# michaelosthege/pytensor-federated

Measured on NVIDIA H100. Metric: logp+grad evals/sec for 8-shard federated GLM, higher is better.
Workload: dtype bf16; 1 GPU; model=federated logistic GLM (logp + gradient), chains_per_eval=1, features=256, global_batch=80000000, seq_len=256, l2_policy=inputs (>= 2.5 GB per GPU) are larger than the 50 MB L2; no flush needed, parallelism=shard-parallel x1 (8 shards/GPU), kernel=auto, backend=fused, comm=local, hbm_bytes_per_eval_per_gpu=31200395264

## Files before the change

### pytensor_federated_b200/csrc/fed_comm.cuh

```cuda
#pragma once
#include <cstdint>
#include <cuda_runtime.h>

#define B200FED_MAX_WORLD 8

#define B200FED_STATUS_SHIFT 56
#define B200FED_EPOCH_MASK 0x00FFFFFFFFFFFFFFull
#define B200FED_ERR_THETA_TIMEOUT 1ull
#define B200FED_ERR_PEER_TIMEOUT 2ull
#define B200FED_ERR_PIPELINE 4ull
#define B200FED_STOP_EPOCH 0x00FFFFFFFFFFFFFFull

struct FedComm {
    int rank;
    int world;
    int n_theta;
    int n_vals;
    unsigned long long epoch;
    unsigned long long timeout_ns;

    const float* theta_src;
    float* peer_theta[B200FED_MAX_WORLD];
    unsigned long long* peer_flag[B200FED_MAX_WORLD];
    float* mc_theta;
// ... 215 lines not shown
        return rl;
    }
    if (c.rank == 0 && blockIdx.x == 0) {
        for (int i = threadIdx.x; i < c.n_theta; i += blockDim.x) {
            float v = c.theta_src[i];
            if (c.mc_theta) {
                multimem_st_f32(c.mc_theta + i, v);
            } else {
                for (int p = 0; p < c.world; ++p) c.peer_theta[p][i] = v;
            }
        }
        __threadfence_system();
        __syncthreads();
        if (threadIdx.x == 0 && c.trace) c.trace[(epoch & 255) * 4 + 0] = globaltimer();
        if (c.mc_flag) {
            if (threadIdx.x == 0) multimem_st_release_u64(c.mc_flag, epoch);
        } else if (threadIdx.x < c.world) {
            st_release_sys(c.peer_flag[threadIdx.x], epoch);
        }
    }
    if (threadIdx.x == 0) {
        unsigned long long seen = 0;
        s_ok = wait_epoch(c.flag_local, epoch, c.timeout_ns, &seen) ? 1 : 0;
        s_seen = seen;
    }
    __syncthreads();
    Prologue r;
    r.epoch = epoch;
    r.timed_out = (s_ok == 0);
    r.stop = ((s_seen & B200FED_EPOCH_MASK) == B200FED_STOP_EPOCH);
    if (!r.timed_out && !r.stop) {
        for (int i = threadIdx.x; i < c.n_theta; i += blockDim.x) theta_smem[i] = ld_cg_f32(c.theta_local + i);
    }
    __syncthreads();
    if (threadIdx.x == 0) stamp(c, 1);
    return r;
}

__device__ __forceinline__ void dd_add(double& hi, double& lo, double xh, double xl) {
    const double s = hi + xh;
    const double bb = s - hi;
    const double err = (hi - (s - bb)) + (xh - bb);
    hi = s;
    lo += err + xl;
}
__device__ __forceinline__ double2 ld_cg_f64x2(const double* p) {
    double2 v;
    asm volatile("ld.global.cg.v2.f64 {%0, %1}, [%2];" : "=d"(v.x), "=d"(v.y) : "l"(p) : "memory");
    return v;
}

constexpr unsigned int kReduceGroup = 16;

template <bool DD>
__device__ __forceinline__ void sum_rows(const double* rows, size_t stride, int v, unsigned int first, unsigned int count,
                                         double& hi, double& lo) {
    constexpr unsigned int kWide = DD ? 16 : 37;
    hi = 0.0;
    lo = 0.0;
    for (unsigned int b = 0; b < count; b += kWide) {
        if constexpr (DD) {
            double2 t[kWide];
#pragma unroll
            for (unsigned int j = 0; j < kWide; ++j)
                t[j] = (b + j < count) ? ld_cg_f64x2(rows + (size_t)(first + b + j) * stride + 2 * (size_t)v) : make_double2(0.0, 0.0);
#pragma unroll
            for (unsigned int j = 0; j < kWide; ++j) dd_add(hi, lo, t[j].x, t[j].y);
        } else {
            double t[kWide];
#pragma unroll
            for (unsigned int j = 0; j < kWide; ++j)
                t[j] = (b + j < count) ? ld_cg_f64(rows + (size_t)(first + b + j) * stride + v) : 0.0;
#pragma unroll
            for (unsigned int j = 0; j < kWide; ++j) hi += t[j];
        }
    }
}

template <bool DD>
__device__ __forceinline__ bool epilogue_t(const FedComm& c, const Prologue& pro, unsigned long long status_in,
                                           size_t row_stride, double* group_buf) {
    __shared__ int s_last;
    __shared__ unsigned long long s_status;
    const int nv = c.n_vals;
    if (c.world == 1 && gridDim.x == 1) {
        __syncthreads();
        if (pro.timed_out || pro.stop) {
            if (threadIdx.x == 0) {
                if (pro.timed_out && !pro.stop && c.spec_theta && c.idle_ticks) {
                    volatile unsigned long long* ticks = c.idle_ticks;
                    *ticks = *ticks + 1ull;
                } else if (c.host_flag) {
                    __threadfence_system();
                    st_release_sys(c.host_flag, (pro.stop ? B200FED_STOP_EPOCH : pro.epoch) |
                                                    ((pro.stop ? 0ull : B200FED_ERR_THETA_TIMEOUT) << B200FED_STATUS_SHIFT));
                }
            }
            return true;
        }
        auto value = [&](int v) { return DD ? c.cta_partials[2 * v] + c.cta_partials[2 * v + 1] : c.cta_partials[v]; };
        if (c.ll_mode) {
            for (int v = threadIdx.x; v < nv; v += blockDim.x) ll_store_f64(c.ll_host_result + 2 * v, value(v), pro.epoch);
            if (threadIdx.x == 0) {
                if (c.trace) {
                    c.trace[(pro.epoch & 255) * 4 + 1] = globaltimer();
                    c.trace[(pro.epoch & 255) * 4 + 2] = globaltimer();
                }
                if (c.epoch_counter) *c.epoch_counter = pro.epoch;
                if (c.done_flag) *reinterpret_cast<volatile unsigned long long*>(c.done_flag) = pro.epoch;
                stamp(c, 7);
            }
            return true;
        }
        for (int v = threadIdx.x; v < nv; v += blockDim.x) c.host_result[v] = value(v);
        __threadfence_system();
        __syncthreads();
        if (threadIdx.x == 0) {
            if (c.trace) {
                c.trace[(pro.epoch & 255) * 4 + 1] = globaltimer();
                c.trace[(pro.epoch & 255) * 4 + 2] = globaltimer();
            }
            st_release_sys(c.host_flag, pro.epoch | (status_in << B200FED_STATUS_SHIFT));
            if (c.epoch_counter) *c.epoch_counter = pro.epoch;
            if (c.done_flag) *reinterpret_cast<volatile unsigned long long*>(c.done_flag) = pro.epoch;
            stamp(c, 7);
        }
        return true;
    }
    const bool computed = !(pro.stop || pro.timed_out);
    const unsigned int n_groups = (gridDim.x + kReduceGroup - 1) / kReduceGroup;
    const unsigned int grp = blockIdx.x / kReduceGroup;
    const unsigned int grp_first = grp * kReduceGroup;
    const unsigned int grp_size = min(kReduceGroup, gridDim.x - grp_first);
    constexpr int kW = DD ? 2 : 1;

    const unsigned long long status_cta = status_in | ((pro.timed_out && !pro.stop) ? B200FED_ERR_THETA_TIMEOUT : 0ull);
    if (threadIdx.x == 0 && status_cta) atomicOr(c.ticket + 255, (unsigned int)status_cta);
    __threadfence();
    __syncthreads();
    if (threadIdx.x == 0) {
        const unsigned int t = atomicAdd(c.ticket + 1 + grp, 1u);
        s_last = (t == grp_size - 1) ? 1 : 0;
        if (s_last) c.ticket[1 + grp] = 0;
        s_status = status_in;
    }
    __syncthreads();
    if (!s_last) {
        if (threadIdx.x == 0) stamp(c, 7);
        return false;
    }
    __threadfence();
    if (computed) {
        for (int v = threadIdx.x; v < nv; v += blockDim.x) {
            double hi, lo;
            sum_rows<DD>(c.cta_partials, row_stride, v, grp_first, grp_size, hi, lo);
            group_buf[((size_t)grp * nv + v) * kW] = hi;
            if constexpr (DD) group_buf[((size_t)grp * nv + v) * kW + 1] = lo;
        }
    }
    __threadfence();
    __syncthreads();
    if (threadIdx.x == 0) {
        const unsigned int t = atomicAdd(c.ticket, 1u);
        s_last = (t == n_groups - 1) ? 1 : 0;
    }
    __syncthreads();
    if (!s_last) {
        if (threadIdx.x == 0) stamp(c, 7);
        return false;
    }
    __threadfence();
    const unsigned long long epoch = pro.epoch;
    if (threadIdx.x == 0) {
        s_status |= (unsigned long long)atomicExch(c.ticket + 255, 0u);
    }
    __syncthreads();
    const bool any_timed_out = (s_status & B200FED_ERR_THETA_TIMEOUT) != 0ull;

    if (!computed || any_timed_out) {
        if (threadIdx.x == 0) {
            const bool timed_out = pro.timed_out || any_timed_out;
            const bool idle = timed_out && !pro.stop && (c.rank != 0 || c.spec_theta != nullptr);
            if (idle && c.rank == 0) *c.spec_abort = 0ull;
            const unsigned long long done_epoch = idle ? epoch - 1ull : epoch;
            *c.ticket = 0;
            if (c.epoch_counter) *c.epoch_counter = done_epoch;
            unsigned long long st = (timed_out && !idle) ? B200FED_ERR_THETA_TIMEOUT : 0ull;
            unsigned long long word = (pro.stop ? B200FED_STOP_EPOCH : done_epoch) | (st << B200FED_STATUS_SHIFT);
            if (idle && c.idle_ticks) {
                volatile unsigned long long* ticks = c.idle_ticks;
                *ticks = *ticks + 1ull;
            }
            if (c.done_flag) { *reinterpret_cast<volatile unsigned long long*>(c.done_flag) = word; }
            if (c.rank == 0 && c.host_flag) {
                __threadfence_system();
                st_release_sys(c.host_flag, word);
            }
        }
        return true;
    }
    auto node_value = [&](int v) {
        double hi, lo;
        sum_rows<DD>(group_buf, (size_t)nv * kW, v, 0u, n_groups, hi, lo);
        return hi + lo;
    };

    if (c.ll_mode) {
        unsigned long long* my_slot_ll = c.ll_root_slots + (size_t)c.rank * nv * 2;
        for (int v = threadIdx.x; v < nv; v += blockDim.x) {
            const double s = node_value(v);
            if (c.rank != 0) {
                ll_store_f64(my_slot_ll + 2 * v, s, epoch);
            } else {
                double total = s;
                bool ok = true;
                for (int p = 1; p < c.world && ok; ++p) {
                    unsigned int lo = 0, hi = 0;
                    const unsigned long long* src = c.ll_root_slots + ((size_t)p * nv + v) * 2;
                    ok = ll_wait_word(src, epoch, c.timeout_ns, nullptr, &lo) == 0 &&
                         ll_wait_word(src + 1, epoch, c.timeout_ns, nullptr, &hi) == 0;
                    total += __longlong_as_double((long long)(((unsigned long long)hi << 32) | lo));
                }
                if (ok) ll_store_f64(c.ll_host_result + 2 * v, total, epoch);
                else atomicOr(&s_status, B200FED_ERR_PEER_TIMEOUT);
            }
        }
        __syncthreads();
        if (threadIdx.x == 0) {
            if (c.trace) {
                c.trace[(epoch & 255) * 4 + 1] = globaltimer();
                if (c.rank == 0) c.trace[(epoch & 255) * 4 + 2] = globaltimer();
            }
            if (c.rank == 0 && s_status) {
                __threadfence_system();
                st_release_sys(c.host_flag, epoch | (s_status << B200FED_STATUS_SHIFT));
            }
            *c.ticket = 0;
            if (c.epoch_counter) *c.epoch_counter = epoch;
            if (c.done_flag) *reinterpret_cast<volatile unsigned long long*>(c.done_flag) = epoch | (s_status << B200FED_STATUS_SHIFT);
            stamp(c, 7);
        }
        return true;
    }

    if (c.rank != 0) {
        double* my_slot = c.root_slots + (size_t)c.rank * nv;
        for (int v = threadIdx.x; v < nv; v += blockDim.x) my_slot[v] = node_value(v);
        __threadfence_system();
        __syncthreads();
        if (threadIdx.x == 0) {
            if (c.trace) c.trace[(epoch & 255) * 4 + 1] = globaltimer();
            st_release_sys(c.root_slot_flags + c.rank, epoch);
        }
    } else {
        if (threadIdx.x == 0 && c.trace) c.trace[(epoch & 255) * 4 + 1] = globaltimer();
        constexpr int kOwn = 4;
// ... 72 lines not shown
```

### pytensor_federated_b200/csrc/glm_tc.cu

```cuda
#include <cstring>
#include <vector>

#include <cuda.h>
#include <cuda_bf16.h>
#include <cuda_runtime.h>

#include "fed_comm.cuh"
#include "models.h"
#include "tc_common.cuh"
#include "chunks.h"

namespace tc {

constexpr int kTileM = 128;
constexpr int kPanel = 64;
constexpr int kPanelBytes = kTileM * 128;
constexpr int kThreads = 384;
constexpr int kConsumerWarps = 8;
constexpr int kMaxChunk = 32;
constexpr int kMinChunk = 4;
constexpr int kRing = 16;
constexpr int kLLRows = 16;

constexpr int kXBlock = kTileM * kPanel * 3 / 2;
constexpr int kXFoot = 256;
constexpr int kXMaxExceptions = kXFoot / 4 - 1;
constexpr int kXSlots = 6;
constexpr int kDecThreads = 96;

__host__ __device__ __forceinline__ uint32_t x12_prmt(uint32_t a, uint32_t b, uint32_t s) {
#ifdef __CUDA_ARCH__
    uint32_t r;
    asm("prmt.b32 %0, %1, %2, %3;" : "=r"(r) : "r"(a), "r"(b), "r"(s));
    return r;
#else
    const uint64_t v = (uint64_t)b << 32 | a;
    uint32_t r = 0;
    for (int k = 0; k < 4; ++k) {
        const uint32_t sel = (s >> (4 * k)) & 0xFu;
        uint32_t byte = (uint32_t)(v >> (8 * (sel & 7u))) & 0xFFu;
        if (sel & 8u) byte = (byte & 0x80u) ? 0xFFu : 0u;
        r |= byte << (8 * k);
    }
    return r;
#endif
}
__host__ __device__ __forceinline__ uint4 x12_decode8(uint2 lo, uint32_t c, const uint32_t (&t)[4]) {
    const uint32_t w = c << 4;
    const uint32_t s0 = c & 0x7777u, s1 = (c >> 16) & 0x7777u;
    const uint32_t m0 = x12_prmt(w, c, 0xD9C8u), m1 = x12_prmt(w, c, 0xFBEAu);
    const uint32_t h0 = (x12_prmt(t[0], t[1], s0) & ~m0) | (x12_prmt(t[2], t[3], s0) & m0);
    const uint32_t h1 = (x12_prmt(t[0], t[1], s1) & ~m1) | (x12_prmt(t[2], t[3], s1) & m1);
    uint4 r;
    r.x = x12_prmt(lo.x, h0, 0x5140u);
    r.y = x12_prmt(lo.x, h0, 0x7362u);
    r.z = x12_prmt(lo.y, h1, 0x5140u);
    r.w = x12_prmt(lo.y, h1, 0x7362u);
    return r;
}
__host__ __device__ __forceinline__ uint32_t x12_chunk_offset(int i) { return (i >> 3) * 128 + (((i & 7) ^ ((i >> 3) & 7)) << 4); }
__host__ __device__ __forceinline__ uint32_t x12_high_byte_offset(uint32_t pos) {
    const uint32_t pnl = pos >> 13, row = (pos >> 6) & 127, f = pos & 63;
    return pnl * kPanelBytes + row * 128 + ((((f >> 3) ^ (row & 7)) << 4) | ((f & 7) << 1)) + 1;
}

struct SmemLayout {
    uint32_t stages, stage_bytes, off_theta_b, theta_b_bytes, off_r, r_bytes, off_rows, row_bytes, off_theta_f,
        off_disp, off_ring, off_bars, total, preload, xslots, xslot_bytes, off_x, off_xfoot;
};
__host__ __device__ inline SmemLayout smem_layout(int P, int n1, int n2, int n_theta, int chain_words, int chains,
                                                  int row_arrays, bool packed = false) {
    SmemLayout L;
    const uint32_t panels = P / kPanel;
    L.stage_bytes = panels * kPanelBytes;
    L.theta_b_bytes = panels * n1 * 128;
    L.r_bytes = kTileM * n2 * 2;
    L.row_bytes = (uint32_t)row_arrays * kTileM * 4;
    const uint32_t bars_bytes = packed ? 256 : 192;
    const uint32_t fixed = L.theta_b_bytes + 2 * L.r_bytes + ((chains * (1 + chain_words) * 4 + 15) & ~15) + kRing * 24 +
                           bars_bytes + (packed ? 2 * kXFoot : 0) + 1024 ;
    uint32_t stages = (227u * 1024u - fixed) / (L.stage_bytes + L.row_bytes);
// ... 156 lines not shown
            if (ROWS && segs_g[i].weight) tma_prefetch_desc(&tmaps[4 * i + 3]);
        }
    auto load_tile = [&](int st, int seg, int row0, int rows) {
        const CUtensorMap* m = tmaps + 4 * seg;
        float* slot = reinterpret_cast<float*>(smem + L.off_rows + (size_t)st * L.row_bytes);
        mbar_expect_tx(&bar_full[st], L.stage_bytes + kTileM * 4 * (1 + (rows & 1) + (rows >> 1)));
        for (int pnl = 0; pnl < panels; ++pnl)
            tma_load_2d(smem + (size_t)st * L.stage_bytes + pnl * kPanelBytes, m, pnl * kPanel, row0, &bar_full[st]);
        tma_load_1d(slot, m + 1, row0, &bar_full[st]);
        if (rows & 1) tma_load_1d(slot + o_slot * kTileM, m + 2, row0, &bar_full[st]);
        if (rows & 2) tma_load_1d(slot + w_slot * kTileM, m + 3, row0, &bar_full[st]);
    };
    auto load_xpanel = [&](int xs, int seg, int tile, int pnl, int rows) {
        unsigned char* dst = smem + L.off_x + (size_t)xs * L.xslot_bytes;
        const GlmSegment& g = segs_g[seg];
        const uint32_t extra = pnl == 0 ? kXFoot + kTileM * 4 * (1 + (rows & 1) + (rows >> 1)) : 0;
        mbar_expect_tx(&bar_xfull[xs], kXBlock + extra);
        bulk_load(dst, static_cast<const unsigned char*>(g.xpack) + ((size_t)tile * panels + pnl) * kXBlock, kXBlock, &bar_xfull[xs]);
        if (pnl == 0) {
            const CUtensorMap* m = tmaps + 4 * seg;
            float* slot = reinterpret_cast<float*>(dst + kXBlock + kXFoot);
            bulk_load(dst + kXBlock, static_cast<const unsigned char*>(g.xfoot) + (size_t)tile * kXFoot, kXFoot, &bar_xfull[xs]);
            tma_load_1d(slot, m + 1, tile * kTileM, &bar_xfull[xs]);
            if (rows & 1) tma_load_1d(slot + o_slot * kTileM, m + 2, tile * kTileM, &bar_xfull[xs]);
            if (rows & 2) tma_load_1d(slot + w_slot * kTileM, m + 3, tile * kTileM, &bar_xfull[xs]);
        }
    };
    auto seg_row_mask = [&](int seg) -> int {
        if constexpr (!ROWS) return 0;
        return (segs_g[seg].offset ? 1 : 0) | (segs_g[seg].weight ? 2 : 0);
    };
    unsigned int claim0 = 0;
    int preloaded = 0;
    if (warp == 0) {
        __syncwarp();
        fed::pdl_wait();
        if (lane == 0) claim0 = atomicAdd(work_counter, 1u);
        claim0 = __shfl_sync(0xffffffffu, claim0, 0);
        if (claim0 < (unsigned int)n_chunks) {
            const GlmChunk ch = chunks[claim0];
            const int units = PK ? ch.n_tiles * panels : ch.n_tiles;
            preloaded = units < (int)L.preload ? units : (int)L.preload;
            if (!prm.early_loads) preloaded = 0;
            const int rows = seg_row_mask(ch.seg);
            if (elect_one())
                for (int t = 0; t < preloaded; ++t) {
                    if (PK) load_xpanel(t, ch.seg, ch.first_tile + t / panels, t % panels, rows);
                    else load_tile(t, ch.seg, (ch.first_tile + t) * kTileM, rows);
                }
            __syncwarp();
        }
    }

    fed::Prologue pro = fed::prologue(comm, theta_f);
    const bool active = !pro.stop && !pro.timed_out;
    const int NOUT = prm.n_out;
    const int NS1 = 1 + G + DISP;
    const size_t row_doubles = partial_row_doubles(comm.n_vals, KC, NOUT, G, DISP);
    double* out = comm.cta_partials + (size_t)blockIdx.x * row_doubles;
    const size_t sum_doubles = partial_sum_doubles(comm.n_vals, KC, NOUT, G, DISP);
    float* icpt_table = reinterpret_cast<float*>(out + sum_doubles);
    double* ll_slots = out + 2 * (size_t)comm.n_vals;

    if (active) {
        for (size_t i = threadIdx.x; i < sum_doubles / 2; i += blockDim.x) reinterpret_cast<double2*>(out)[i] = make_double2(0.0, 0.0);
        for (int i = threadIdx.x; i < KC * G; i += blockDim.x)
            icpt_table[i] = (i / G) < nch ? theta_f[(i / G) * (G + P + DISP) + (i % G)] : 0.f;
        if constexpr (DISP)
            for (int k = threadIdx.x; k < KC; k += blockDim.x)
                chain_constants<E>(prm.family, k < nch ? theta_f[k * (G + P + 1) + G + P] : 0.f, disp + k * kDispWords);
        for (int idx = threadIdx.x; idx < panels * N1 * 8; idx += blockDim.x) {
            const int j = idx & 7;
            const int n = (idx >> 3) % N1;
            const int pnl = idx / (8 * N1);
            const int chain = n % C8, term = n / C8;
            uint32_t packed[4] = {0, 0, 0, 0};
            if (chain < nch) {
#pragma unroll
                for (int e = 0; e < 8; ++e) {
                    const int f = pnl * kPanel + j * 8 + e;
                    const float v = f < P ? theta_f[chain * (G + P + DISP) + G + f] : 0.f;
                    const __nv_bfloat16 hi = __float2bfloat16_rn(v);
                    const float rem1 = v - __bfloat162float(hi);
                    const __nv_bfloat16 mid = __float2bfloat16_rn(rem1);
                    const __nv_bfloat16 lo = __float2bfloat16_rn(rem1 - __bfloat162float(mid));
                    const __nv_bfloat16 pick = term == 0 ? hi : (term == 1 ? mid : lo);
                    const uint32_t bits = (uint32_t)__bfloat16_as_ushort(pick);
                    packed[e >> 1] |= bits << ((e & 1) * 16);
                }
            }
            uint4* dst = reinterpret_cast<uint4*>(theta_b + pnl * (N1 * 128) + n * 128 + ((j ^ (n & 7)) * 16));
            *dst = make_uint4(packed[0], packed[1], packed[2], packed[3]);
        }
        fence_proxy_async();
        __syncthreads();
        if (threadIdx.x == 0) fed::stamp(comm, 2);

        auto next_chunk = [&](int j) -> int4 {
            mbar_wait(&bar_ring[j & (kRing - 1)], (uint32_t)((j / kRing) & 1));
            if (*pipeline_fault()) return make_int4(-1, 0, 0, 0);
            return ring[j & (kRing - 1)];
        };
        int4* chunk_decided = reinterpret_cast<int4*>(smem + L.off_bars + 128);
        auto consumer_chunk = [&](int j) -> int4 {
            const int slot = j & (kRing - 1);
            mbar_wait(&bar_ring[slot], (uint32_t)((j / kRing) & 1));
            named_sync(1, 256);
            if (threadIdx.x == 128) *chunk_decided = *pipeline_fault() ? make_int4(-1, 0, 0, 0) : ring[slot];
            if (threadIdx.x >= 128 && threadIdx.x < 128 + KC && !*pipeline_fault() && ring[slot].x >= 0)
                icpt[threadIdx.x - 128] = __ldcg(icpt_table + (threadIdx.x - 128) * G + ring[slot].w);
            named_sync(1, 256);
            return *chunk_decided;
        };

        if (warp == 0) {
            Ring stage, xs;
            unsigned int claim = claim0, ahead = 0;
            for (int j = 0;; ++j) {
                const bool have = claim < (unsigned int)n_chunks;
                GlmChunk ch{};
                if (have) ch = chunks[claim];
                if (lane == 0) {
                    ring[j & (kRing - 1)] = have ? make_int4(ch.seg, ch.first_tile * kTileM, ch.n_tiles, segs_g[ch.seg].group)
                                                 : make_int4(-1, 0, 0, 0);
                    mbar_arrive(&bar_ring[j & (kRing - 1)]);
                    if (have) ahead = atomicAdd(work_counter, 1u);
                }
                __syncwarp();
                if (!have) break;
                const int rows = seg_row_mask(ch.seg);
                for (int t = 0; t < ch.n_tiles && PK; ++t)
                    for (int pnl = 0; pnl < panels; ++pnl) {
                        const int k = t * panels + pnl;
                        if (!(j == 0 && k < preloaded)) {
                            mbar_wait(&bar_xempty[xs.idx], xs.phase ^ 1);
                            if (j == 0 && k == preloaded && lane == 0) fed::stamp(comm, 3);
                            if (elect_one()) load_xpanel(xs.idx, ch.seg, ch.first_tile + t, pnl, rows);
                            __syncwarp();
                        }
                        xs.advance((int)L.xslots);
                    }
                for (int t = 0; t < ch.n_tiles && !PK; ++t) {
                    const int st = stage.idx;
                    if (j == 0 && t < preloaded) {
                        stage.advance(S);
                        continue;
                    }
                    mbar_wait(&bar_empty[st], stage.phase ^ 1);
                    if (j == 0 && t == preloaded && lane == 0) fed::stamp(comm, 3);
                    if (elect_one()) load_tile(st, ch.seg, (ch.first_tile + t) * kTileM, rows);
                    __syncwarp();
                    stage.advance(S);
                }
                claim = __shfl_sync(0xffffffffu, ahead, 0);
            }
            if (lane == 0) fed::stamp(comm, 4);
        } else if (warp < 4) {
            if (PK) {
                const int td = threadIdx.x - 32;
                constexpr int kDecGroup = KC <= 4 && traits(E).group_panels ? 2 : 1;
                static_assert(kDecGroup <= 2, "a packed launch may have only 2 compressed slots");
                int4* decided = reinterpret_cast<int4*>(smem + L.off_bars + 144);
                Ring stage, xs;
                uint32_t fb = 0;
                for (int j = 0;; ++j) {
                    mbar_wait(&bar_ring[j & (kRing - 1)], (uint32_t)((j / kRing) & 1));
                    named_sync(2, kDecThreads);
                    if (td == 0) *decided = *pipeline_fault() ? make_int4(-1, 0, 0, 0) : ring[j & (kRing - 1)];
                    named_sync(2, kDecThreads);
                    const int4 ch = *decided;
                    if (ch.x < 0) break;
                    const uint32_t tab[4] = {segs_g[ch.x].xtab[0], segs_g[ch.x].xtab[1], segs_g[ch.x].xtab[2],
                                             segs_g[ch.x].xtab[3]};
                    for (int t = 0; t < ch.z; ++t) {
                        mbar_wait(&bar_empty[stage.idx], stage.phase ^ 1);
                        unsigned char* dst = smem + (size_t)stage.idx * L.stage_bytes;
                        int* foot = reinterpret_cast<int*>(smem + L.off_xfoot + fb * kXFoot);
                        for (int pnl = 0; pnl < panels; pnl += kDecGroup) {
                            constexpr int kPer = (kTileM * 8 + kDecThreads - 1) / kDecThreads;
                            uint2 lo[kDecGroup][kPer];
                            uint32_t cw[kDecGroup][kPer];
                            int xi[kDecGroup];
#pragma unroll
                            for (int h = 0; h < kDecGroup; ++h) {
                                mbar_wait(&bar_xfull[xs.idx], xs.phase);
                                const unsigned char* src = smem + L.off_x + (size_t)xs.idx * L.xslot_bytes;
                                if (pnl + h == 0) {
                                    if (td < kXFoot / 4) foot[td] = reinterpret_cast<const int*>(src + kXBlock)[td];
                                    const float* rsrc = reinterpret_cast<const float*>(src + kXBlock + kXFoot);
                                    float* rdst = reinterpret_cast<float*>(smem + L.off_rows + (size_t)stage.idx * L.row_bytes);
                                    for (int i = td; i < (int)L.row_bytes / 4; i += kDecThreads) rdst[i] = rsrc[i];
                                }
#pragma unroll
                                for (int k = 0; k < kPer; ++k) {
                                    const int i = td + k * kDecThreads;
                                    if (k < kPer - 1 || i < kTileM * 8) {
                                        lo[h][k] = reinterpret_cast<const uint2*>(src)[i];
                                        cw[h][k] = reinterpret_cast<const uint32_t*>(src + kTileM * kPanel)[i];
                                    }
                                }
                                xi[h] = xs.idx;
                                xs.advance((int)L.xslots);
                            }
#pragma unroll
                            for (int h = 0; h < kDecGroup; ++h) {
                                unsigned char* pd = dst + (pnl + h) * kPanelBytes;
#pragma unroll
                                for (int k = 0; k < kPer; ++k) {
                                    const int i = td + k * kDecThreads;
                                    if (k < kPer - 1 || i < kTileM * 8)
                                        *reinterpret_cast<uint4*>(pd + x12_chunk_offset(i)) = x12_decode8(lo[h][k], cw[h][k], tab);
                                }
                                mbar_arrive(&bar_xempty[xi[h]]);
                            }
                        }
                        named_sync(2, kDecThreads);
                        const int n_ex = min(foot[0], kXMaxExceptions);
                        for (int e = td; e < n_ex; e += kDecThreads) {
                            const uint32_t v = (uint32_t)foot[1 + e];
                            if ((v >> 8) < (uint32_t)panels * kTileM * kPanel) dst[x12_high_byte_offset(v >> 8)] = (unsigned char)(v & 0xFFu);
                        }
                        fence_proxy_async();
                        mbar_arrive(&bar_full[stage.idx]);
                        stage.advance(S);
                        fb ^= 1u;
                    }
                }
            }
        } else {
            const int c = (warp >> 2) - 1;
            const int w = warp & 3;
            const int q = lane & 3;
            const int ew = warp - 4;
            const int NB = PP / 128;
            constexpr int NJ = C8 / 8;
            const uint64_t desc_k = make_desc(0, 16, 1024, 1);
            const uint64_t desc_xt = make_desc(0, kPanelBytes, 1024, 1);
            const uint64_t desc_r = make_desc(0, 128, 2048, 0);
            const uint32_t theta_b_a = smem_u32(theta_b);
            const uint32_t x_base_a = smem_u32(smem);
            const uint32_t r_a = smem_u32(r_buf);
            float gacc[3][N2 / 2];
#pragma unroll
            for (int i = 0; i < 3; ++i)
#pragma unroll
                for (int v = 0; v < N2 / 2; ++v) gacc[i][v] = 0.f;
            int sm_chain[2 * NJ];
            float sm_cls[2 * NJ];
            int sm_chains = 0;
            if constexpr (SOFTMAX) {
                const int NC = prm.n_classes;
                sm_chains = nch / NC;
#pragma unroll
                for (int s = 0; s < 2 * NJ; ++s) {
                    const int v = 8 * (s >> 1) + 2 * q + (s & 1);
                    sm_chain[s] = v < nch ? v / NC : -1;
                    sm_cls[s] = (float)(v % NC);
                }
            }
            int od_chain[2 * NJ], od_cut[2 * NJ];
            int od_chains = 0, od_ncut = 1;
            if constexpr (ORD) {
                od_ncut = prm.n_classes - 1;
                od_chains = nch / od_ncut;
#pragma unroll
                for (int s = 0; s < 2 * NJ; ++s) {
                    const int v = 8 * (s >> 1) + 2 * q + (s & 1);
                    od_chain[s] = v < nch ? v / od_ncut : -1;
                    od_cut[s] = v % od_ncut;
                }
            }
            Ring stage;
            uint32_t rb = 0;
            for (int j = 0;; ++j) {
                const int4 ch = consumer_chunk(j);
                if (ch.x < 0) break;
                const bool has_o = ROWS && segs_g[ch.x].offset != nullptr;
                const bool has_w = ROWS && segs_g[ch.x].weight != nullptr;
                const long long seg_rows = segs_g[ch.x].n_rows;
                const int seg_group = segs_g[ch.x].group;
                const int og = segs_g[ch.x].out_group;
                float ll_acc[2 * NJ], gi_acc[2 * NJ], ds_acc[2 * NJ];
// ... 196 lines not shown
                                            hv_h = link_curvature(fam, et);
                                            if constexpr (ROWS) {
                                                apply_weight(wt, ll);
                                                apply_weight(wt, r);
                                            }
                                        } else {
                                            r = __fmul_rn(hv_h, eta + icpt[k]);
                                            if constexpr (ROWS) apply_weight(wt, r);
                                        }
                                    } else if constexpr (ROWS) {
                                        link_loglik(prm.family, y, __fadd_rn(eta + icpt[k], o), ll, r);
                                        apply_weight(wt, ll);
                                        apply_weight(wt, r);
                                    } else {
                                        link_loglik(prm.family, y, eta + icpt[k], ll, r);
                                    }
                                }
                                ll_acc[2 * jc + e] += ll;
                                gi_acc[2 * jc + e] += r;
                                if constexpr (DISP) ds_acc[2 * jc + e] += dq;
                                if (k < N2 / 2) {
                                    const __nv_bfloat16 hi = __float2bfloat16_rn(r);
                                    const __nv_bfloat16 lo = __float2bfloat16_rn(r - __bfloat162float(hi));
                                    unsigned char* p0 = rbuf + ((2 * k) / 8) * 2048 + (row / 8) * 128 + (row % 8) * 2;
                                    *reinterpret_cast<__nv_bfloat16*>(p0 + ((2 * k) % 8) * 16) = hi;
                                    *reinterpret_cast<__nv_bfloat16*>(p0 + ((2 * k + 1) % 8) * 16) = lo;
                                }
                            }
                        }
                        }
                    }
                    fence_proxy_async();
                    named_sync(1, 32 * kConsumerWarps);
                    wgmma_fence();
#pragma unroll
                    for (int i = 0; i < 3; ++i)
                        if (i < NB) {
                            const uint32_t xa = x_a + (c * NB + i) * kPanelBytes;
#pragma unroll
                            for (int ks = 0; ks < kTileM / 16; ++ks) {
                                const uint64_t adesc = desc_xt | (uint64_t)((xa + ks * 2048) >> 4);
                                const uint64_t bdesc = desc_r | (uint64_t)((r_a + rb * L.r_bytes + ks * 256) >> 4);
                                wgmma_bf16<N2, 1, 0>(gacc[i], adesc, bdesc, (t | ks) ? 1u : 0u);
                            }
                        }
                    wgmma_commit();
                    wgmma_wait<0>();
#pragma unroll
                    for (int i = 0; i < 3; ++i) fence_regs(gacc[i]);
                    mbar_arrive(&bar_empty[stage.idx]);
                    stage.advance(S);
                    rb ^= 1u;
                }
#pragma unroll
                for (int s = 0; s < 2 * NJ; ++s) {
                    double lsum = (double)ll_acc[s], gsum = (double)gi_acc[s], dsum = (double)ds_acc[s];
#pragma unroll
                    for (int o = 4; o < 32; o <<= 1) {
                        lsum += __shfl_xor_sync(0xffffffffu, lsum, o);
                        gsum += __shfl_xor_sync(0xffffffffu, gsum, o);
                        if constexpr (DISP) dsum += __shfl_xor_sync(0xffffffffu, dsum, o);
                    }
                    const int k = 8 * (s >> 1) + 2 * q + (s & 1);
                    if (lane < 4 && k < nch) {
                        double* slot = ll_slots + 2 * ((((size_t)ew * NOUT + og) * KC + k) * NS1);
                        dd_accumulate(slot, lsum);
                        dd_accumulate(slot + 2 * (1 + seg_group), gsum);
                        if constexpr (DISP) dd_accumulate(slot + 2 * (1 + G), dsum);
                    }
                }
#pragma unroll
                for (int i = 0; i < 3; ++i)
                    if (i < NB) {
#pragma unroll
                        for (int jn = 0; jn < N2 / 8; ++jn)
#pragma unroll
                            for (int h = 0; h < 2; ++h) {
                                const int f = 64 * (c * NB + i) + 16 * w + (lane >> 2) + 8 * h;
                                const int k = 4 * jn + q;
                                if (k < nch && f < P)
                                    dd_accumulate(out + 2 * (((size_t)og * nch + k) * NV1 + 1 + G + f),
                                                  (double)gacc[i][4 * jn + 2 * h] + (double)gacc[i][4 * jn + 2 * h + 1]);
                            }
                    }
            }
        }

        __syncthreads();
        fed::pdl_trigger();
        if (threadIdx.x == 0) fed::stamp(comm, 5);
        for (int i = threadIdx.x; i < NOUT * nch * NS1; i += blockDim.x) {
            const int j = i % NS1, k = (i / NS1) % nch, o = i / (NS1 * nch);
            double hi = 0.0, lo = 0.0;
            for (int w = 0; w < kConsumerWarps; ++w) {
                const double* slot = ll_slots + 2 * ((((size_t)w * NOUT + o) * KC + k) * NS1 + j);
                fed::dd_add(hi, lo, slot[0], slot[1]);
            }
            const int jo = (DISP && j == 1 + G) ? 1 + G + P : j;
            out[2 * (((size_t)o * nch + k) * NV1 + jo)] = hi;
            out[2 * (((size_t)o * nch + k) * NV1 + jo) + 1] = lo;
        }
        if (threadIdx.x == 0) fed::stamp(comm, 6);
    } else if (warp == 0) {
        for (int t = 0; t < preloaded; ++t) mbar_wait(PK ? &bar_xfull[t] : &bar_full[t], 0u);
    }
    __syncthreads();
    const unsigned long long status = *pipeline_fault() ? B200FED_ERR_PIPELINE : 0ull;
    const bool fin = fed::epilogue_t<true>(comm, pro, status, row_doubles, comm.group_partials);
    if (fin && threadIdx.x == 0) *work_counter = 0u;
}

}

namespace {
int chains_bucket(int k) { return k <= 1 ? 1 : (k <= 4 ? 4 : (k <= 8 ? 8 : (k <= 16 ? 16 : 0))); }

tc::SmemLayout launch_layout(int n_features, int kc, tc::Epi e, int n_theta, bool rows, int row_data, bool packed = false) {
    return tc::smem_layout((n_features + 127) & ~127, tc::cfg(kc).N1, tc::cfg(kc).N2, n_theta,
                           tc::traits(e).disp ? tc::kDispWords : 0, kc, tc::row_arrays(rows, row_data), packed);
}

using LaunchFn = int (*)(const FedComm*, const GlmSegment*, const GlmParams*, const void*, const void*, int, unsigned int*,
                         int, cudaStream_t);

template <int KC, bool ROWS, tc::Epi E>
int launch(const FedComm* comm, const GlmSegment* segs_dev, const GlmParams* prm, const void* tmaps, const void* chunks_dev,
           int n_chunks, unsigned int* work_counter, int grid, cudaStream_t stream) {
    const tc::SmemLayout L = launch_layout(prm->n_features, KC, E, comm->n_theta, ROWS, prm->row_data, prm->packed_x != 0);
    if (L.stages < 2) return -2;
    if (prm->packed_x && L.xslots < 2) return -4;
    return tc::launch_pdl(tc::fed_glm_tc_kernel<KC, ROWS, E>, grid, tc::kThreads, L.total, stream, *comm, segs_dev, *prm,
                          reinterpret_cast<const CUtensorMap*>(tmaps), reinterpret_cast<const GlmChunk*>(chunks_dev),
                          n_chunks, work_counter);
}

template <tc::Epi E>
LaunchFn pick(int kc, bool rows) {
    switch (kc) {
        case 1:
            if constexpr (tc::traits(E).two_columns) return nullptr;
            else return rows ? launch<1, true, E> : launch<1, false, E>;
        case 4: return rows ? launch<4, true, E> : launch<4, false, E>;
        case 8: return rows ? launch<8, true, E> : launch<8, false, E>;
        default: return rows ? launch<16, true, E> : launch<16, false, E>;
    }
}
LaunchFn pick(tc::Epi e, int kc, bool rows) {
    using tc::Epi;
    switch (e) {
        case Epi::Hvp: return pick<Epi::Hvp>(kc, rows);
        case Epi::Softmax: return pick<Epi::Softmax>(kc, rows);
        case Epi::Ordinal: return pick<Epi::Ordinal>(kc, rows);
        case Epi::Survival: return pick<Epi::Survival>(kc, rows);
        case Epi::Dispersion: return pick<Epi::Dispersion>(kc, rows);
        default: return pick<Epi::Scalar>(kc, rows);
        case Epi::ZeroInflated: return pick<Epi::ZeroInflated>(kc, rows);
        case Epi::ZeroInflatedDisp: return pick<Epi::ZeroInflatedDisp>(kc, rows);
        case Epi::Positive: return pick<Epi::Positive>(kc, rows);
        case Epi::LocationScale: return pick<Epi::LocationScale>(kc, rows);
        case Epi::StudentT: return pick<Epi::StudentT>(kc, rows);
        case Epi::Beta: return pick<Epi::Beta>(kc, rows);
// ... 115 lines not shown
```

### pytensor_federated_b200/csrc/tc_common.cuh

```cuda
#pragma once
#include <cstdlib>

#include <cuda.h>
#include <cuda_bf16.h>
#include <cuda_runtime.h>
#include <cudaTypedefs.h>

#include "fed_comm.cuh"
#include "glm_link.cuh"
#include "models.h"

namespace tc {

__device__ __forceinline__ uint32_t smem_u32(const void* p) { return (uint32_t)__cvta_generic_to_shared(p); }

__device__ __forceinline__ void mbar_init(uint64_t* bar, uint32_t count) {
    asm volatile("mbarrier.init.shared::cta.b64 [%0], %1;" ::"r"(smem_u32(bar)), "r"(count));
}
__device__ __forceinline__ void mbar_arrive(uint64_t* bar) {
    asm volatile("mbarrier.arrive.shared::cta.b64 _, [%0];" ::"r"(smem_u32(bar)) : "memory");
}
__device__ __forceinline__ void mbar_expect_tx(uint64_t* bar, uint32_t bytes) {
    asm volatile("mbarrier.arrive.expect_tx.shared::cta.b64 _, [%0], %1;" ::"r"(smem_u32(bar)), "r"(bytes) : "memory");
}
// ... 15 lines not shown
    return &fault;
}
__device__ __forceinline__ void mbar_wait(uint64_t* bar, uint32_t parity) {
    if (mbar_try_wait(bar, parity)) return;
    const unsigned long long t0 = fed::globaltimer();
    volatile int* fault = pipeline_fault();
    while (!mbar_try_wait(bar, parity)) {
        if (*fault) return;
        if (fed::globaltimer() - t0 > 4000000000ull) {
            *fault = 1;
            return;
        }
    }
}
__device__ __forceinline__ bool elect_one() {
    uint32_t pred;
    asm volatile(
        "{\n\t"
        ".reg .pred p;\n\t"
        "elect.sync _|p, 0xffffffff;\n\t"
        "selp.u32 %0, 1, 0, p;\n\t"
        "}"
        : "=r"(pred));
    return pred != 0;
}
__device__ __forceinline__ void fence_barrier_init() { asm volatile("fence.mbarrier_init.release.cluster;" ::: "memory"); }
__device__ __forceinline__ void fence_proxy_async() { asm volatile("fence.proxy.async.shared::cta;" ::: "memory"); }

__device__ __forceinline__ void tma_load_2d(void* smem_dst, const CUtensorMap* map, int c0, int c1, uint64_t* bar) {
    asm volatile(
        "cp.async.bulk.tensor.2d.shared::cluster.global.mbarrier::complete_tx::bytes [%0], [%1, {%2, %3}], [%4];" ::"r"(
            smem_u32(smem_dst)),
        "l"(map), "r"(c0), "r"(c1), "r"(smem_u32(bar))
        : "memory");
}
__device__ __forceinline__ void tma_load_1d(void* smem_dst, const CUtensorMap* map, int c0, uint64_t* bar) {
    asm volatile(
        "cp.async.bulk.tensor.1d.shared::cluster.global.mbarrier::complete_tx::bytes [%0], [%1, {%2}], [%3];" ::"r"(
            smem_u32(smem_dst)),
        "l"(map), "r"(c0), "r"(smem_u32(bar))
        : "memory");
}
__device__ __forceinline__ void bulk_load(void* smem_dst, const void* src, uint32_t bytes, uint64_t* bar) {
    asm volatile(
        "cp.async.bulk.shared::cluster.global.mbarrier::complete_tx::bytes [%0], [%1], %2, [%3];" ::"r"(smem_u32(smem_dst)),
        "l"(src), "r"(bytes), "r"(smem_u32(bar))
        : "memory");
}
__device__ __forceinline__ void tma_prefetch_desc(const CUtensorMap* map) {
    asm volatile("prefetch.tensormap [%0];" ::"l"(map) : "memory");
}

__device__ __forceinline__ void named_sync(int id, int count) { asm volatile("bar.sync %0, %1;" ::"r"(id), "r"(count) : "memory"); }

__device__ __forceinline__ void wgmma_fence() { asm volatile("wgmma.fence.sync.aligned;" ::: "memory"); }
__device__ __forceinline__ void wgmma_commit() { asm volatile("wgmma.commit_group.sync.aligned;" ::: "memory"); }
template <int N>
__device__ __forceinline__ void wgmma_wait() { asm volatile("wgmma.wait_group.sync.aligned %0;" ::"n"(N) : "memory"); }
template <int N>
__device__ __forceinline__ void fence_regs(float (&d)[N]) {
#pragma unroll
    for (int i = 0; i < N; ++i) asm volatile("" : "+f"(d[i])::"memory");
}

template <int N, int TA, int TB>
__device__ __forceinline__ void wgmma_bf16(float (&d)[N / 2], uint64_t adesc, uint64_t bdesc, uint32_t scale_d) {
    static_assert(N == 8 || N == 16 || N == 24 || N == 32 || N == 48, "instantiated widths");
    if constexpr (N == 8) {
        asm volatile(
            "{\n\t.reg .pred p;\n\tsetp.ne.b32 p, %6, 0;\n\t"
            "wgmma.mma_async.sync.aligned.m64n8k16.f32.bf16.bf16 {%0, %1, %2, %3}, %4, %5, p, 1, 1, %7, %8;\n\t}"
            : "+f"(d[0]), "+f"(d[1]), "+f"(d[2]), "+f"(d[3])
            : "l"(adesc), "l"(bdesc), "r"(scale_d), "n"(TA), "n"(TB));
    } else if constexpr (N == 16) {
        asm volatile(
            "{\n\t.reg .pred p;\n\tsetp.ne.b32 p, %10, 0;\n\t"
            "wgmma.mma_async.sync.aligned.m64n16k16.f32.bf16.bf16 {%0, %1, %2, %3, %4, %5, %6, %7}, %8, %9, p, 1, 1, %11, %12;\n\t}"
            : "+f"(d[0]), "+f"(d[1]), "+f"(d[2]), "+f"(d[3]), "+f"(d[4]), "+f"(d[5]), "+f"(d[6]), "+f"(d[7])
            : "l"(adesc), "l"(bdesc), "r"(scale_d), "n"(TA), "n"(TB));
    } else if constexpr (N == 24) {
        asm volatile(
            "{\n\t.reg .pred p;\n\tsetp.ne.b32 p, %14, 0;\n\t"
            "wgmma.mma_async.sync.aligned.m64n24k16.f32.bf16.bf16 {%0, %1, %2, %3, %4, %5, %6, %7, %8, %9, %10, %11}, %12, %13, p, 1, 1, %15, %16;\n\t}"
            : "+f"(d[0]), "+f"(d[1]), "+f"(d[2]), "+f"(d[3]), "+f"(d[4]), "+f"(d[5]), "+f"(d[6]), "+f"(d[7]), "+f"(d[8]), "+f"(d[9]), "+f"(d[10]), "+f"(d[11])
            : "l"(adesc), "l"(bdesc), "r"(scale_d), "n"(TA), "n"(TB));
    } else if constexpr (N == 32) {
        asm volatile(
            "{\n\t.reg .pred p;\n\tsetp.ne.b32 p, %18, 0;\n\t"
            "wgmma.mma_async.sync.aligned.m64n32k16.f32.bf16.bf16 {%0, %1, %2, %3, %4, %5, %6, %7, %8, %9, %10, %11, %12, %13, %14, %15}, %16, %17, p, 1, 1, %19, %20;\n\t}"
            : "+f"(d[0]), "+f"(d[1]), "+f"(d[2]), "+f"(d[3]), "+f"(d[4]), "+f"(d[5]), "+f"(d[6]), "+f"(d[7]), "+f"(d[8]), "+f"(d[9]), "+f"(d[10]), "+f"(d[11]), "+f"(d[12]), "+f"(d[13]), "+f"(d[14]), "+f"(d[15])
            : "l"(adesc), "l"(bdesc), "r"(scale_d), "n"(TA), "n"(TB));
    } else if constexpr (N == 48) {
        asm volatile(
            "{\n\t.reg .pred p;\n\tsetp.ne.b32 p, %26, 0;\n\t"
            "wgmma.mma_async.sync.aligned.m64n48k16.f32.bf16.bf16 {%0, %1, %2, %3, %4, %5, %6, %7, %8, %9, %10, %11, %12, %13, %14, %15, %16, %17, %18, %19, %20, %21, %22, %23}, %24, %25, p, 1, 1, %27, %28;\n\t}"
            : "+f"(d[0]), "+f"(d[1]), "+f"(d[2]), "+f"(d[3]), "+f"(d[4]), "+f"(d[5]), "+f"(d[6]), "+f"(d[7]), "+f"(d[8]), "+f"(d[9]), "+f"(d[10]), "+f"(d[11]), "+f"(d[12]), "+f"(d[13]), "+f"(d[14]), "+f"(d[15]), "+f"(d[16]), "+f"(d[17]), "+f"(d[18]), "+f"(d[19]), "+f"(d[20]), "+f"(d[21]), "+f"(d[22]), "+f"(d[23])
            : "l"(adesc), "l"(bdesc), "r"(scale_d), "n"(TA), "n"(TB));
    }
}

template <int N>
__device__ __forceinline__ void wgmma_e4m3(float (&d)[N / 2], uint64_t adesc, uint64_t bdesc, uint32_t scale_d) {
    static_assert(N == 32 || N == 40, "instantiated widths");
    if constexpr (N == 32) {
        asm volatile(
            "{\n\t.reg .pred p;\n\tsetp.ne.b32 p, %18, 0;\n\t"
// ... 581 lines not shown
```

Measured before the change: 87.79 evals/s.

## Add a fourth warpgroup for decode and rebalance registers with setmaxnreg

Raises the block from 384 to 512 threads, adding four warps (12-15) that join warps 1-3 in decompressing packed X panels, so the decoder group grows from 96 to 224 threads. setmaxnreg then gives the producer and decoder warps 88 registers and the wgmma consumer warps 168. Pointer and prologue values are recomputed from opaque values or kept in shared memory to cut register pressure, and the DD reduction width drops to 12. The aim is more decode throughput without register spills in the consumers. The risk is that the larger block lowers the launch register budget to 128 per thread, and a consumer capped at 168 could spill.

```diff
diff --git a/pytensor_federated_b200/csrc/fed_comm.cuh b/pytensor_federated_b200/csrc/fed_comm.cuh
--- a/pytensor_federated_b200/csrc/fed_comm.cuh
+++ b/pytensor_federated_b200/csrc/fed_comm.cuh
@@ -291,10 +291,10 @@
 
 constexpr unsigned int kReduceGroup = 16;
 
-template <bool DD>
+template <bool DD, unsigned int kWideDD = 16>
 __device__ __forceinline__ void sum_rows(const double* rows, size_t stride, int v, unsigned int first, unsigned int count,
                                          double& hi, double& lo) {
-    constexpr unsigned int kWide = DD ? 16 : 37;
+    constexpr unsigned int kWide = DD ? kWideDD : 37;
     hi = 0.0;
     lo = 0.0;
     for (unsigned int b = 0; b < count; b += kWide) {
@@ -316,7 +316,7 @@
     }
 }
 
-template <bool DD>
+template <bool DD, unsigned int kWideDD = 16>
 __device__ __forceinline__ bool epilogue_t(const FedComm& c, const Prologue& pro, unsigned long long status_in,
                                            size_t row_stride, double* group_buf) {
     __shared__ int s_last;
@@ -392,7 +392,7 @@
     if (computed) {
         for (int v = threadIdx.x; v < nv; v += blockDim.x) {
             double hi, lo;
-            sum_rows<DD>(c.cta_partials, row_stride, v, grp_first, grp_size, hi, lo);
+            sum_rows<DD, kWideDD>(c.cta_partials, row_stride, v, grp_first, grp_size, hi, lo);
             group_buf[((size_t)grp * nv + v) * kW] = hi;
             if constexpr (DD) group_buf[((size_t)grp * nv + v) * kW + 1] = lo;
         }
@@ -440,7 +440,7 @@
     }
     auto node_value = [&](int v) {
         double hi, lo;
-        sum_rows<DD>(group_buf, (size_t)nv * kW, v, 0u, n_groups, hi, lo);
+        sum_rows<DD, kWideDD>(group_buf, (size_t)nv * kW, v, 0u, n_groups, hi, lo);
         return hi + lo;
     };
 
diff --git a/pytensor_federated_b200/csrc/glm_tc.cu b/pytensor_federated_b200/csrc/glm_tc.cu
--- a/pytensor_federated_b200/csrc/glm_tc.cu
+++ b/pytensor_federated_b200/csrc/glm_tc.cu
@@ -15,7 +15,11 @@
 constexpr int kTileM = 128;
 constexpr int kPanel = 64;
 constexpr int kPanelBytes = kTileM * 128;
-constexpr int kThreads = 384;
+constexpr int kThreads = 512;
+constexpr int kRegs = 65536 / kThreads;
+constexpr int kConsumerRegs = 168;
+constexpr int kOtherRegs = 88;
+static_assert(256 * kConsumerRegs + 256 * kOtherRegs == 65536, "the register split must fill the register file");
 constexpr int kConsumerWarps = 8;
 constexpr int kMaxChunk = 32;
 constexpr int kMinChunk = 4;
@@ -26,7 +30,7 @@
 constexpr int kXFoot = 256;
 constexpr int kXMaxExceptions = kXFoot / 4 - 1;
 constexpr int kXSlots = 6;
-constexpr int kDecThreads = 96;
+constexpr int kDecThreads = 224;
 
 __host__ __device__ __forceinline__ uint32_t x12_prmt(uint32_t a, uint32_t b, uint32_t s) {
 #ifdef __CUDA_ARCH__
@@ -289,20 +293,31 @@
         }
     }
 
-    fed::Prologue pro = fed::prologue(comm, theta_f);
-    const bool active = !pro.stop && !pro.timed_out;
+    __shared__ fed::Prologue s_pro;
+    bool active;
+    {
+        const fed::Prologue pro = fed::prologue(comm, theta_f);
+        if (threadIdx.x == 0) s_pro = pro;
+        active = !pro.stop && !pro.timed_out;
+    }
     const int NOUT = prm.n_out;
     const int NS1 = 1 + G + DISP;
-    const size_t row_doubles = partial_row_doubles(comm.n_vals, KC, NOUT, G, DISP);
-    double* out = comm.cta_partials + (size_t)blockIdx.x * row_doubles;
-    const size_t sum_doubles = partial_sum_doubles(comm.n_vals, KC, NOUT, G, DISP);
-    float* icpt_table = reinterpret_cast<float*>(out + sum_doubles);
-    double* ll_slots = out + 2 * (size_t)comm.n_vals;
+    auto row_doubles = [&] { return partial_row_doubles(opaque(comm.n_vals), KC, NOUT, G, DISP); };
+    auto cta_row = [&]() -> double* { return comm.cta_partials + (size_t)blockIdx.x * row_doubles(); };
+    auto icpt_table = [&]() -> float* {
+        return reinterpret_cast<float*>(cta_row() + partial_sum_doubles(opaque(comm.n_vals), KC, NOUT, G, DISP));
+    };
+    auto ll_slots = [&]() -> double* { return cta_row() + 2 * (size_t)opaque(comm.n_vals); };
 
     if (active) {
-        for (size_t i = threadIdx.x; i < sum_doubles / 2; i += blockDim.x) reinterpret_cast<double2*>(out)[i] = make_double2(0.0, 0.0);
+        {
+            double* out = cta_row();
+            const size_t sum_doubles = partial_sum_doubles(comm.n_vals, KC, NOUT, G, DISP);
+            for (size_t i = threadIdx.x; i < sum_doubles / 2; i += blockDim.x) reinterpret_cast<double2*>(out)[i] = make_double2(0.0, 0.0);
+        }
+        float* const itab = icpt_table();
         for (int i = threadIdx.x; i < KC * G; i += blockDim.x)
-            icpt_table[i] = (i / G) < nch ? theta_f[(i / G) * (G + P + DISP) + (i % G)] : 0.f;
+            itab[i] = (i / G) < nch ? theta_f[(i / G) * (G + P + DISP) + (i % G)] : 0.f;
         if constexpr (DISP)
             for (int k = threadIdx.x; k < KC; k += blockDim.x)
                 chain_constants<E>(prm.family, k < nch ? theta_f[k * (G + P + 1) + G + P] : 0.f, disp + k * kDispWords);
@@ -345,126 +360,132 @@
             named_sync(1, 256);
             if (threadIdx.x == 128) *chunk_decided = *pipeline_fault() ? make_int4(-1, 0, 0, 0) : ring[slot];
             if (threadIdx.x >= 128 && threadIdx.x < 128 + KC && !*pipeline_fault() && ring[slot].x >= 0)
-                icpt[threadIdx.x - 128] = __ldcg(icpt_table + (threadIdx.x - 128) * G + ring[slot].w);
+                icpt[threadIdx.x - 128] = __ldcg(icpt_table() + (threadIdx.x - 128) * G + ring[slot].w);
             named_sync(1, 256);
             return *chunk_decided;
         };
 
-        if (warp == 0) {
-            Ring stage, xs;
-            unsigned int claim = claim0, ahead = 0;
-            for (int j = 0;; ++j) {
-                const bool have = claim < (unsigned int)n_chunks;
-                GlmChunk ch{};
-                if (have) ch = chunks[claim];
-                if (lane == 0) {
-                    ring[j & (kRing - 1)] = have ? make_int4(ch.seg, ch.first_tile * kTileM, ch.n_tiles, segs_g[ch.seg].group)
-                                                 : make_int4(-1, 0, 0, 0);
-                    mbar_arrive(&bar_ring[j & (kRing - 1)]);
-                    if (have) ahead = atomicAdd(work_counter, 1u);
+        if (warp < 4 || warp >= 12) {
+            setmaxnreg<kRegs, kOtherRegs>();
+            if (warp == 0) {
+                Ring stage, xs;
+                unsigned int claim = claim0, ahead = 0;
+                for (int j = 0;; ++j) {
+                    const bool have = claim < (unsigned int)n_chunks;
+                    GlmChunk ch{};
+                    if (have) ch = chunks[claim];
+                    if (lane == 0) {
+                        ring[j & (kRing - 1)] = have ? make_int4(ch.seg, ch.first_tile * kTileM, ch.n_tiles, segs_g[ch.seg].group)
+                                                     : make_int4(-1, 0, 0, 0);
+                        mbar_arrive(&bar_ring[j & (kRing - 1)]);
+                        if (have) ahead = atomicAdd(work_counter, 1u);
+                    }
+                    __syncwarp();
+                    if (!have) break;
+                    const int rows = seg_row_mask(ch.seg);
+                    for (int t = 0; t < ch.n_tiles && PK; ++t)
+                        for (int pnl = 0; pnl < panels; ++pnl) {
+                            const int k = t * panels + pnl;
+                            if (!(j == 0 && k < preloaded)) {
+                                mbar_wait(&bar_xempty[xs.idx], xs.phase ^ 1);
+                                if (j == 0 && k == preloaded && lane == 0) fed::stamp(comm, 3);
+                                if (elect_one()) load_xpanel(xs.idx, ch.seg, ch.first_tile + t, pnl, rows);
+                                __syncwarp();
+                            }
+                            xs.advance((int)L.xslots);
+                        }
+                    for (int t = 0; t < ch.n_tiles && !PK; ++t) {
+                        const int st = stage.idx;
+                        if (j == 0 && t < preloaded) {
+                            stage.advance(S);
+                            continue;
+                        }
+                        mbar_wait(&bar_empty[st], stage.phase ^ 1);
+                        if (j == 0 && t == preloaded && lane == 0) fed::stamp(comm, 3);
+                        if (elect_one()) load_tile(st, ch.seg, (ch.first_tile + t) * kTileM, rows);
+                        __syncwarp();
+                        stage.advance(S);
+                    }
+                    claim = __shfl_sync(0xffffffffu, ahead, 0);
                 }
-                __syncwarp();
-                if (!have) break;
-                const int rows = seg_row_mask(ch.seg);
-                for (int t = 0; t < ch.n_tiles && PK; ++t)
-                    for (int pnl = 0; pnl < panels; ++pnl) {
-                        const int k = t * panels + pnl;
-                        if (!(j == 0 && k < preloaded)) {
-                            mbar_wait(&bar_xempty[xs.idx], xs.phase ^ 1);
-                            if (j == 0 && k == preloaded && lane == 0) fed::stamp(comm, 3);
-                            if (elect_one()) load_xpanel(xs.idx, ch.seg, ch.first_tile + t, pnl, rows);
-                            __syncwarp();
-                        }
-                        xs.advance((int)L.xslots);
-                    }
-                for (int t = 0; t < ch.n_tiles && !PK; ++t) {
-                    const int st = stage.idx;
-                    if (j == 0 && t < preloaded) {
-                        stage.advance(S);
-                        continue;
-                    }
-                    mbar_wait(&bar_empty[st], stage.phase ^ 1);
-                    if (j == 0 && t == preloaded && lane == 0) fed::stamp(comm, 3);
-                    if (elect_one()) load_tile(st, ch.seg, (ch.first_tile + t) * kTileM, rows);
-                    __syncwarp();
-                    stage.advance(S);
-                }
-                claim = __shfl_sync(0xffffffffu, ahead, 0);
-            }
-            if (lane == 0) fed::stamp(comm, 4);
-        } else if (warp < 4) {
-            if (PK) {
-                const int td = threadIdx.x - 32;
-                constexpr int kDecGroup = KC <= 4 && traits(E).group_panels ? 2 : 1;
-                static_assert(kDecGroup <= 2, "a packed launch may have only 2 compressed slots");
-                int4* decided = reinterpret_cast<int4*>(smem + L.off_bars + 144);
-                Ring stage, xs;
-                uint32_t fb = 0;
-                for (int j = 0;; ++j) {
-                    mbar_wait(&bar_ring[j & (kRing - 1)], (uint32_t)((j / kRing) & 1));
-                    named_sync(2, kDecThreads);
-                    if (td == 0) *decided = *pipeline_fault() ? make_int4(-1, 0, 0, 0) : ring[j & (kRing - 1)];
-                    named_sync(2, kDecThreads);
-                    const int4 ch = *decided;
-                    if (ch.x < 0) break;
-                    const uint32_t tab[4] = {segs_g[ch.x].xtab[0], segs_g[ch.x].xtab[1], segs_g[ch.x].xtab[2],
-                                             segs_g[ch.x].xtab[3]};
-                    for (int t = 0; t < ch.z; ++t) {
-                        mbar_wait(&bar_empty[stage.idx], stage.phase ^ 1);
-                        unsigned char* dst = smem + (size_t)stage.idx * L.stage_bytes;
-                        int* foot = reinterpret_cast<int*>(smem + L.off_xfoot + fb * kXFoot);
-                        for (int pnl = 0; pnl < panels; pnl += kDecGroup) {
-                            constexpr int kPer = (kTileM * 8 + kDecThreads - 1) / kDecThreads;
-                            uint2 lo[kDecGroup][kPer];
-                            uint32_t cw[kDecGroup][kPer];
-                            int xi[kDecGroup];
-#pragma unroll
-                            for (int h = 0; h < kDecGroup; ++h) {
-                                mbar_wait(&bar_xfull[xs.idx], xs.phase);
-                                const unsigned char* src = smem + L.off_x + (size_t)xs.idx * L.xslot_bytes;
-                                if (pnl + h == 0) {
-                                    if (td < kXFoot / 4) foot[td] = reinterpret_cast<const int*>(src + kXBlock)[td];
-                                    const float* rsrc = reinterpret_cast<const float*>(src + kXBlock + kXFoot);
-                                    float* rdst = reinterpret_cast<float*>(smem + L.off_rows + (size_t)stage.idx * L.row_bytes);
-                                    for (int i = td; i < (int)L.row_bytes / 4; i += kDecThreads) rdst[i] = rsrc[i];
+                if (lane == 0) fed::stamp(comm, 4);
+            } else {
+                if (PK) {
+                    const int td = warp < 4 ? threadIdx.x - 32 : threadIdx.x - (12 * 32 - 96);
+                    constexpr int kDecGroup = KC <= 4 && traits(E).group_panels ? 2 : 1;
+                    static_assert(kDecGroup <= 2, "a packed launch may have only 2 compressed slots");
+                    int4* decided = reinterpret_cast<int4*>(smem + L.off_bars + 144);
+                    Ring stage, xs;
+                    uint32_t fb = 0;
+                    for (int j = 0;; ++j) {
+                        mbar_wait(&bar_ring[j & (kRing - 1)], (uint32_t)((j / kRing) & 1));
+                        named_sync(2, kDecThreads);
+                        if (td == 0) *decided = *pipeline_fault() ? make_int4(-1, 0, 0, 0) : ring[j & (kRing - 1)];
+                        named_sync(2, kDecThreads);
+                        const int4 ch = *decided;
+                        if (ch.x < 0) break;
+                        const uint32_t tab[4] = {segs_g[ch.x].xtab[0], segs_g[ch.x].xtab[1], segs_g[ch.x].xtab[2],
+                                                 segs_g[ch.x].xtab[3]};
+                        for (int t = 0; t < ch.z; ++t) {
+                            mbar_wait(&bar_empty[stage.idx], stage.phase ^ 1);
+                            unsigned char* dst = smem + (size_t)stage.idx * L.stage_bytes;
+                            int* foot = reinterpret_cast<int*>(smem + L.off_xfoot + fb * kXFoot);
+                            for (int pnl = 0; pnl < panels; pnl += kDecGroup) {
+                                constexpr int kPer = (kTileM * 8 + kDecThreads - 1) / kDecThreads;
+                                uint2 lo[kDecGroup][kPer];
+                                uint32_t cw[kDecGroup][kPer];
+                                int xi[kDecGroup];
+#pragma unroll
+                                for (int h = 0; h < kDecGroup; ++h) {
+                                    mbar_wait(&bar_xfull[xs.idx], xs.phase);
+                                    const unsigned char* src = smem + L.off_x + (size_t)xs.idx * L.xslot_bytes;
+                                    if (pnl + h == 0) {
+                                        if (td < kXFoot / 4) foot[td] = reinterpret_cast<const int*>(src + kXBlock)[td];
+                                        const float* rsrc = reinterpret_cast<const float*>(src + kXBlock + kXFoot);
+                                        float* rdst = reinterpret_cast<float*>(smem + L.off_rows + (size_t)stage.idx * L.row_bytes);
+                                        for (int i = td; i < (int)L.row_bytes / 4; i += kDecThreads) rdst[i] = rsrc[i];
+                                    }
+#pragma unroll
+                                    for (int k = 0; k < kPer; ++k) {
+                                        const int i = td + k * kDecThreads;
+                                        if (k < kPer - 1 || i < kTileM * 8) {
+                                            lo[h][k] = reinterpret_cast<const uint2*>(src)[i];
+                                            cw[h][k] = reinterpret_cast<const uint32_t*>(src + kTileM * kPanel)[i];
+                                        }
+                                    }
+                                    xi[h] = xs.idx;
+                                    xs.advance((int)L.xslots);
                                 }
 #pragma unroll
-                                for (int k = 0; k < kPer; ++k) {
-                                    const int i = td + k * kDecThreads;
-                                    if (k < kPer - 1 || i < kTileM * 8) {
-                                        lo[h][k] = reinterpret_cast<const uint2*>(src)[i];
-                                        cw[h][k] = reinterpret_cast<const uint32_t*>(src + kTileM * kPanel)[i];
+                                for (int h = 0; h < kDecGroup; ++h) {
+                                    unsigned char* pd = dst + (pnl + h) * kPanelBytes;
+#pragma unroll
+                                    for (int k = 0; k < kPer; ++k) {
+                                        const int i = td + k * kDecThreads;
+                                        if (k < kPer - 1 || i < kTileM * 8)
+                                            *reinterpret_cast<uint4*>(pd + x12_chunk_offset(i)) = x12_decode8(lo[h][k], cw[h][k], tab);
                                     }
+                                    mbar_arrive(&bar_xempty[xi[h]]);
                                 }
-                                xi[h] = xs.idx;
-                                xs.advance((int)L.xslots);
                             }
-#pragma unroll
-                            for (int h = 0; h < kDecGroup; ++h) {
-                                unsigned char* pd = dst + (pnl + h) * kPanelBytes;
-#pragma unroll
-                                for (int k = 0; k < kPer; ++k) {
-                                    const int i = td + k * kDecThreads;
-                                    if (k < kPer - 1 || i < kTileM * 8)
-                                        *reinterpret_cast<uint4*>(pd + x12_chunk_offset(i)) = x12_decode8(lo[h][k], cw[h][k], tab);
-                                }
-                                mbar_arrive(&bar_xempty[xi[h]]);
+                            named_sync(2, kDecThreads);
+                            const int n_ex = min(foot[0], kXMaxExceptions);
+                            for (int e = td; e < n_ex; e += kDecThreads) {
+                                const uint32_t v = (uint32_t)foot[1 + e];
+                                if ((v >> 8) < (uint32_t)panels * kTileM * kPanel) dst[x12_high_byte_offset(v >> 8)] = (unsigned char)(v & 0xFFu);
                             }
-                        }
-                        named_sync(2, kDecThreads);
-                        const int n_ex = min(foot[0], kXMaxExceptions);
-                        for (int e = td; e < n_ex; e += kDecThreads) {
-                            const uint32_t v = (uint32_t)foot[1 + e];
-                            if ((v >> 8) < (uint32_t)panels * kTileM * kPanel) dst[x12_high_byte_offset(v >> 8)] = (unsigned char)(v & 0xFFu);
-                        }
-                        fence_proxy_async();
-                        mbar_arrive(&bar_full[stage.idx]);
-                        stage.advance(S);
-                        fb ^= 1u;
+                            fence_proxy_async();
+                            mbar_arrive(&bar_full[stage.idx]);
+                            stage.advance(S);
+                            fb ^= 1u;
+                        }
                     }
                 }
             }
+            named_sync(3, kThreads);
+            setmaxnreg<kOtherRegs, kRegs>();
         } else {
+            setmaxnreg<kRegs, kConsumerRegs>();
             const int c = (warp >> 2) - 1;
             const int w = warp & 3;
             const int q = lane & 3;
@@ -767,6 +788,8 @@
                     stage.advance(S);
                     rb ^= 1u;
                 }
+                double* const out = cta_row();
+                double* const slots = out + 2 * (size_t)comm.n_vals;
 #pragma unroll
                 for (int s = 0; s < 2 * NJ; ++s) {
                     double lsum = (double)ll_acc[s], gsum = (double)gi_acc[s], dsum = (double)ds_acc[s];
@@ -778,7 +801,7 @@
                     }
                     const int k = 8 * (s >> 1) + 2 * q + (s & 1);
                     if (lane < 4 && k < nch) {
-                        double* slot = ll_slots + 2 * ((((size_t)ew * NOUT + og) * KC + k) * NS1);
+                        double* slot = slots + 2 * ((((size_t)ew * NOUT + og) * KC + k) * NS1);
                         dd_accumulate(slot, lsum);
                         dd_accumulate(slot + 2 * (1 + seg_group), gsum);
                         if constexpr (DISP) dd_accumulate(slot + 2 * (1 + G), dsum);
@@ -799,16 +822,20 @@
                             }
                     }
             }
+            setmaxnreg<kConsumerRegs, kRegs>();
+            named_sync(3, kThreads);
         }
 
         __syncthreads();
         fed::pdl_trigger();
         if (threadIdx.x == 0) fed::stamp(comm, 5);
+        double* const out = cta_row();
+        const double* const slots = ll_slots();
         for (int i = threadIdx.x; i < NOUT * nch * NS1; i += blockDim.x) {
             const int j = i % NS1, k = (i / NS1) % nch, o = i / (NS1 * nch);
             double hi = 0.0, lo = 0.0;
             for (int w = 0; w < kConsumerWarps; ++w) {
-                const double* slot = ll_slots + 2 * ((((size_t)w * NOUT + o) * KC + k) * NS1 + j);
+                const double* slot = slots + 2 * ((((size_t)w * NOUT + o) * KC + k) * NS1 + j);
                 fed::dd_add(hi, lo, slot[0], slot[1]);
             }
             const int jo = (DISP && j == 1 + G) ? 1 + G + P : j;
@@ -821,7 +848,8 @@
     }
     __syncthreads();
     const unsigned long long status = *pipeline_fault() ? B200FED_ERR_PIPELINE : 0ull;
-    const bool fin = fed::epilogue_t<true>(comm, pro, status, row_doubles, comm.group_partials);
+    const fed::Prologue pro = s_pro;
+    const bool fin = fed::epilogue_t<true, 12>(comm, pro, status, row_doubles(), comm.group_partials);
     if (fin && threadIdx.x == 0) *work_counter = 0u;
 }
 
diff --git a/pytensor_federated_b200/csrc/tc_common.cuh b/pytensor_federated_b200/csrc/tc_common.cuh
--- a/pytensor_federated_b200/csrc/tc_common.cuh
+++ b/pytensor_federated_b200/csrc/tc_common.cuh
@@ -91,6 +91,18 @@
 }
 
 __device__ __forceinline__ void named_sync(int id, int count) { asm volatile("bar.sync %0, %1;" ::"r"(id), "r"(count) : "memory"); }
+
+__device__ __forceinline__ int opaque(int v) {
+    asm volatile("" : "+r"(v));
+    return v;
+}
+
+template <int From, int To>
+__device__ __forceinline__ void setmaxnreg() {
+    static_assert(To % 8 == 0 && To >= 24 && To <= 256 && To != From, "setmaxnreg: a multiple of 8 in [24, 256]");
+    if constexpr (To > From) asm volatile("setmaxnreg.inc.sync.aligned.u32 %0;" ::"n"(To));
+    else asm volatile("setmaxnreg.dec.sync.aligned.u32 %0;" ::"n"(To));
+}
 
 __device__ __forceinline__ void wgmma_fence() { asm volatile("wgmma.fence.sync.aligned;" ::: "memory"); }
 __device__ __forceinline__ void wgmma_commit() { asm volatile("wgmma.commit_group.sync.aligned;" ::: "memory"); }
```

After: 96.59 evals/s, median of 6. 1.1x the previous value.
